# DakeQQ/Voice-Activity-Detection-VAD-ONNX

Hardware: NVIDIA B200
Metric: RTFx (audio-hours/sec) (higher is better)
Workload: dtype f32

## Files before the change

voice-activity-detection-vad-onnx_b200/csrc/stft_tc.cu:

```cuda
#include "tc_ptx.cuh"

namespace vadx {

constexpr int kStNPad = 80;
constexpr int kStTerms = 2;
constexpr int kStLead = 8;
constexpr int kStJ = 2;
constexpr int kStSlices = 2 * kStJ;
constexpr int kStStages = 3;
constexpr int kStLoaderWarps = 16;
constexpr int kStOutLd = 44;

struct StftTcArgs {
  const int16_t* X;
  int64_t in_stride;
  int64_t L;
  int64_t S;
  int n_frames, hop;
  int h16;
  int n_q;
  int tq;
  int rows;
  int slice_units;
  int n_st;
  const uint8_t* Wimg;
  float* P;
  int64_t ldp;
  int n_bins, kc, n_k16, n_tiles, vec_p;
  int pad_left;
  const float* mean;
  const int* mean_int;
  const float* dc;
  int n_edge_lo, t_edge_hi;
  float power_scale;
  int stage_out;
  unsigned backoff_ld, backoff_epi;
  int debug;
};

__device__ __forceinline__ uint32_t bf16x2_lo(uint32_t w) {
  const float a = __uint_as_float(0x4B000000u | (w & 0xffu)) - 8388608.0f;
  const float b = __uint_as_float(0x4B000000u | ((w >> 16) & 0xffu)) - 8388608.0f;
  return __byte_perm(__float_as_uint(a), __float_as_uint(b), 0x7632);
}
__device__ __forceinline__ uint32_t bf16x2_hi(uint32_t w) {
  const uint32_t ha = (((w >> 8) & 0xffu) ^ 0x80u);
  const uint32_t hb = (((w >> 24) & 0xffu) ^ 0x80u);
  const float a = fmaf(__uint_as_float(0x4B000000u | ha), 256.0f, -(8388608.0f + 128.0f) * 256.0f);
  const float b = fmaf(__uint_as_float(0x4B000000u | hb), 256.0f, -(8388608.0f + 128.0f) * 256.0f);
  return __byte_perm(__float_as_uint(a), __float_as_uint(b), 0x7632);
}

__device__ __forceinline__ uint32_t f16x2_lo(uint32_t w) {
  const uint32_t m = (w & 0x00ff00ffu) | 0x64006400u;
  uint32_t r;
  asm("sub.rn.f16x2 %0, %1, %2;" : "=r"(r) : "r"(m), "r"(0x64006400u));
  return r;
}
__device__ __forceinline__ uint32_t f16x2_hi(uint32_t w) {
  const uint32_t m = (((w >> 8) & 0x00ff00ffu) ^ 0x00800080u) | 0x64006400u;
  uint32_t r;
  asm("sub.rn.f16x2 %0, %1, %2;" : "=r"(r) : "r"(m), "r"(0x64806480u));
  asm("mul.rn.f16x2 %0, %1, %2;" : "=r"(r) : "r"(r), "r"(0x5c005c00u));
  return r;
}

__device__ __forceinline__ void split17(int d, float& hi, float& lo) {
  lo = __uint_as_float(0x4B000000u | (uint32_t)(d & 255)) - 8388608.0f;
  const uint32_t h = (uint32_t)((d >> 8) + 256);
  hi = fmaf(__uint_as_float(0x4B000000u | h), 256.0f, -(8388608.0f + 256.0f) * 256.0f);
}

template <bool EX, bool F16>
__global__ void __launch_bounds__((kStLoaderWarps + 5) * 32, 1) stft_power_tc_kernel(const StftTcArgs g) {
  constexpr int kStEpiWarp0 = kStLoaderWarps, kStMmaWarp = kStLoaderWarps + 4;
  extern __shared__ __align__(1024) uint8_t smem_raw[];
  uint8_t* w_smem = smem_raw;
  const uint32_t img_bytes = kStNPad * 128u;
  const int w_bytes = g.kc * kStTerms * (int)img_bytes;
  uint8_t* a_smem = w_smem + w_bytes;
  const uint32_t slice_bytes = (uint32_t)g.slice_units * 16u;
  const uint32_t term_bytes = kStSlices * slice_bytes;
  const uint32_t stage_bytes = 2u * term_bytes;
  uint64_t* bars = reinterpret_cast<uint64_t*>(a_smem + (size_t)kStStages * stage_bytes);
  uint32_t* tmem_slot = reinterpret_cast<uint32_t*>(bars + 13);
  float* out_stage = reinterpret_cast<float*>(bars + 16);

  const int warp = threadIdx.x >> 5, lane = threadIdx.x & 31;
  const uint32_t bar0 = smem_u32(bars);
  auto full_bar = [&](int s) { return bar0 + 8u * s; };
  auto empty_bar = [&](int s) { return bar0 + 8u * (4 + s); };
  auto tfull_bar = [&](int b) { return bar0 + 8u * (8 + b); };
  auto tempty_bar = [&](int b) { return bar0 + 8u * (10 + b); };
  const uint32_t wbar = bar0 + 8u * 12;
  constexpr int kAccN = 2 * kStNPad;
  constexpr uint32_t kTmemCols = 512;

  if (threadIdx.x == 0) {
    for (int s = 0; s < kStStages; ++s) {
      mbar_init(full_bar(s), kStLoaderWarps);
      mbar_init(empty_bar(s), 1);
    }
    for (int b = 0; b < 2; ++b) {
      mbar_init(tfull_bar(b), 1);
      mbar_init(tempty_bar(b), 4);
    }
    mbar_init(wbar, 1);
    asm volatile("fence.mbarrier_init.release.cluster;" ::: "memory");
  }
  if (warp == kStMmaWarp) {
    asm volatile("tcgen05.alloc.cta_group::1.sync.aligned.shared::cta.b32 [%0], %1;" ::"r"(smem_u32(tmem_slot)),
                 "r"(kTmemCols)
                 : "memory");
    asm volatile("tcgen05.relinquish_alloc_permit.cta_group::1.sync.aligned;" ::: "memory");
  }
  tc_fence_before();
  __syncthreads();
  tc_fence_after();
  const uint32_t tmem_base = *tmem_slot;
  const int ntile = blockIdx.y;

  if (warp == kStMmaWarp) {
    if (lane == 0) {
      mbar_expect_tx(wbar, (uint32_t)w_bytes);
      const uint8_t* src = g.Wimg + (size_t)ntile * w_bytes;
      for (int t = 0; t < g.kc * kStTerms; ++t) bulk_g2s(smem_u32(w_smem) + t * img_bytes, src + (size_t)t * img_bytes, img_bytes, wbar);
      mbar_wait(wbar, 0);
      const uint32_t idesc = F16 ? umma_idesc_f16(kAccN) : umma_idesc_bf16(kAccN);
      const uint64_t dw = umma_desc_sw128(smem_u32(w_smem));
      const uint64_t da0 = umma_desc_noswz(smem_u32(a_smem), slice_bytes, 128u);
      const uint32_t chunk_units = (kStTerms * img_bytes) >> 4, lo_units = term_bytes >> 4, stage_units = stage_bytes >> 4;
      const uint32_t col_units = (2u * slice_bytes) >> 4;
      const int h16 = g.h16, n_k16 = g.n_k16;
      const uint32_t lo_on = (g.debug & 4) ? 0u : 1u;
      constexpr bool kBurst = F16 && !EX;
      auto b_desc = [&](int k) { return dw + (uint64_t)((uint32_t)(k >> 2) * chunk_units + 2u * (uint32_t)(k & 3)); };
      int stage = 0;
      uint32_t phase = 0;
      int it = 0;
      for (int tile = blockIdx.x; tile < g.n_tiles; tile += gridDim.x, ++it) {
        const int b = it & 1;
        const uint32_t use = (uint32_t)(it >> 1);
        mbar_wait(tempty_bar(b), (use & 1u) ^ 1u);
        tc_fence_after();
        const uint32_t d_tmem = tmem_base + (uint32_t)(b * kAccN);
        for (int st = 0; st < g.n_st; ++st) {
          mbar_wait(full_bar(stage), phase);
          tc_fence_after();
          const uint64_t da_st = da0 + (uint64_t)stage * stage_units;
#pragma unroll
          for (int jj = 0; jj < kStJ; ++jj) {
            const int j = st * kStJ + jj;
            if (j >= h16) break;
            const uint64_t da_j = da_st + (uint64_t)jj * col_units;
            if (kBurst) {
              for (int q0 = 0, k = j; k < n_k16; q0 += 3, k += 3 * h16) {
                const int n_pairs = 1 + (k + h16 < n_k16 ? 1 : 0) + (k + 2 * h16 < n_k16 ? 1 : 0);
                umma_split_x3(d_tmem, da_j + (uint64_t)q0, 1u, lo_units, b_desc(k), b_desc(k + h16), b_desc(k + 2 * h16),
                              idesc, k ? 1u : 0u, n_pairs, lo_on);
              }
            } else {
              for (int q = 0, k = j; k < n_k16; ++q, k += h16) {
                const uint64_t da = da_j + (uint64_t)q;
                if (g.debug & 4) umma_bf16(d_tmem, da, b_desc(k), idesc, k ? 1u : 0u);
                else umma_x2(d_tmem, da, da + lo_units, b_desc(k), idesc, k ? 1u : 0u);
              }
            }
          }
          umma_commit(empty_bar(stage));
          if (++stage == kStStages) { stage = 0; phase ^= 1u; }
        }
        umma_commit(tfull_bar(b));
      }
    }
  } else if (warp < kStLoaderWarps) {
    constexpr int kRowsPerPass = kStLoaderWarps * 32 / kStSlices;
    constexpr int kPasses = 2;
    const int t = threadIdx.x;
    const int sl = t % kStSlices;
    const int r_in = t / kStSlices;
    const int16_t* xs_n[kPasses];
    int h0_n[kPasses];
    uint32_t rok_n = 0u;
    int tile_cached = -1;
    struct Seq { int tile, st; };
    auto valid = [&](const Seq& q) { return q.tile < g.n_tiles; };
    auto advance = [&](Seq& q) { if (++q.st == g.n_st) { q.st = 0; q.tile += gridDim.x; } };
    const int n_groups = 2 * g.h16;
    auto issue = [&](const Seq& q, uint4* raw, uint32_t& msk) {
      msk = 0u;
      if (q.tile != tile_cached) {
        rok_n = 0u;
#pragma unroll
        for (int pass = 0; pass < kPasses; ++pass) {
          const int r = pass * kRowsPerPass + r_in;
          const int64_t slot = (int64_t)q.tile * kTcBM + r;
          const int64_t s = slot / g.tq;
          const int h = (int)(slot - s * g.tq);
          const bool ok = r < g.rows && s < g.S;
          xs_n[pass] = g.X + (ok ? s : 0) * g.in_stride;
          h0_n[pass] = h * g.hop - (EX ? g.pad_left : 0) - kStLead;
          if (ok) rok_n |= 1u << pass;
        }
        tile_cached = q.tile;
      }
      const int grp = q.st * kStSlices + sl;
#pragma unroll
      for (int pass = 0; pass < kPasses; ++pass) {
        const int i0 = h0_n[pass] + 8 * grp;
        uint4 v = make_uint4(0u, 0u, 0u, 0u);
        if (((rok_n >> pass) & 1u) && grp < n_groups && i0 >= 0 && i0 + 7 < g.L) {
          v = __ldg(reinterpret_cast<const uint4*>(xs_n[pass] + i0));
          msk |= 1u << pass;
        }
        raw[pass] = v;
      }
    };
    int stage = 0;
    uint32_t phase = 0;
    int mi_c[kPasses];
#pragma unroll
    for (int pass = 0; pass < kPasses; ++pass) mi_c[pass] = 0;
    int tile_cached_c = -1;
    auto consume = [&](const Seq& q, const uint4* raw, uint32_t msk) {
      if (EX && g.mean_int && q.tile != tile_cached_c) {
#pragma unroll
        for (int pass = 0; pass < kPasses; ++pass) {
          const int64_t s = ((int64_t)q.tile * kTcBM + pass * kRowsPerPass + r_in) / g.tq;
          mi_c[pass] = s < g.S ? __ldg(g.mean_int + s) : 0;
        }
        tile_cached_c = q.tile;
      }
      mbar_wait(empty_bar(stage), phase ^ 1u, g.backoff_ld);
      uint8_t* st_hi = a_smem + (size_t)stage * stage_bytes + sl * slice_bytes;
      uint8_t* st_lo = st_hi + term_bytes;
      if (!(g.debug & 8) && q.st * kStSlices + sl < n_groups)
#pragma unroll
      for (int pass = 0; pass < kPasses; ++pass) {
        const int r = pass * kRowsPerPass + r_in;
        if (r >= g.rows) break;
        const uint32_t wds[4] = {raw[pass].x, raw[pass].y, raw[pass].z, raw[pass].w};
        uint32_t hi[4], lo[4];
        if (EX && g.mean_int) {
          const int mi = ((msk >> pass) & 1u) ? mi_c[pass] : 0;
#pragma unroll
          for (int j = 0; j < 4; ++j) {
            const uint32_t w = wds[j];
            const int a = ((int)(w << 16) >> 16) - mi;
            const int b = ((int)w >> 16) - mi;
            float ah, al, bh, bl;
            split17(a, ah, al);
            split17(b, bh, bl);
            hi[j] = __byte_perm(__float_as_uint(ah), __float_as_uint(bh), 0x7632);
            lo[j] = __byte_perm(__float_as_uint(al), __float_as_uint(bl), 0x7632);
          }
        } else {
#pragma unroll
        for (int j = 0; j < 4; ++j) {
          const uint32_t w = wds[j];
          hi[j] = F16 ? f16x2_hi(w) : bf16x2_hi(w);
          lo[j] = F16 ? f16x2_lo(w) : bf16x2_lo(w);
        }
        }
        *reinterpret_cast<uint4*>(st_hi + r * 16) = make_uint4(hi[0], hi[1], hi[2], hi[3]);
        *reinterpret_cast<uint4*>(st_lo + r * 16) = make_uint4(lo[0], lo[1], lo[2], lo[3]);
      }
      if (!(g.debug & 16)) fence_proxy_async();
      __syncwarp();
      if (lane == 0) mbar_arrive(full_bar(stage));
      if (++stage == kStStages) { stage = 0; phase ^= 1u; }
    };
    constexpr int kStBufs = EX ? 4 : 6;
    uint4 bufs[kStBufs][kPasses];
    uint32_t msks[kStBufs];
#pragma unroll
    for (int i = 0; i < kStBufs; ++i) msks[i] = 0u;
    Seq nxt{(int)blockIdx.x, 0}, cur{(int)blockIdx.x, 0};
#pragma unroll
    for (int i = 0; i < kStBufs - 1; ++i)
      if (valid(nxt)) { issue(nxt, bufs[i], msks[i]); advance(nxt); }
    while (valid(cur)) {
#pragma unroll
      for (int i = 0; i < kStBufs; ++i) {
        constexpr int kPrev = kStBufs - 1;
        if (valid(nxt)) { issue(nxt, bufs[(i + kPrev) % kStBufs], msks[(i + kPrev) % kStBufs]); advance(nxt); }
        consume(cur, bufs[i], msks[i]); advance(cur);
        if (!valid(cur)) break;
      }
    }
  } else {
    const int q = warp - kStEpiWarp0;
    int it = 0;
    const int f0 = ntile * (kStNPad / 2);
    for (int tile = blockIdx.x; tile < g.n_tiles; tile += gridDim.x, ++it) {
      const int b = it & 1;
      const uint32_t use = (uint32_t)(it >> 1);
      mbar_wait(tfull_bar(b), use & 1u, g.backoff_epi);
      tc_fence_after();
      const int64_t slot = (int64_t)tile * kTcBM + q * 32 + lane;
      const int64_t sidx = slot / g.tq;
      const int t = (int)(slot - sidx * g.tq);
      const bool row_ok = sidx < g.S && t < g.n_frames;
      const int64_t row = row_ok ? sidx * g.n_frames + t : -1;
      const uint32_t taddr = tmem_base + ((uint32_t)(q * 32) << 16) + (uint32_t)(b * kAccN);
      float* const my_out = out_stage + (size_t)q * 32 * kStOutLd;
      float m_row = 0.f, x_last = 0.f;
      const float* dc_row = nullptr;
      const float* tail_row = nullptr;
      if (EX && g.dc && row_ok) {
        const int n_edge = g.n_edge_lo + (g.n_frames - g.t_edge_hi);
        if (g.mean) {
          m_row = __ldg(g.mean + sidx);
          const int e = t < g.n_edge_lo ? 1 + t : (t >= g.t_edge_hi ? 1 + g.n_edge_lo + (t - g.t_edge_hi) : 0);
          dc_row = g.dc + ((size_t)e * gridDim.y + ntile) * kStNPad;
        }
        if (t >= g.t_edge_hi) {
          x_last = (float)((int)__ldg(g.X + sidx * g.in_stride + (g.L - 1)) - (g.mean_int ? __ldg(g.mean_int + sidx) : 0));
          tail_row = g.dc + ((size_t)(1 + n_edge + (t - g.t_edge_hi)) * gridDim.y + ntile) * kStNPad;
        }
      }
#pragma unroll
      for (int c0 = 0; c0 < kStNPad; c0 += 16) {
        float v[16], v2[16];
        tmem_ld16(taddr + (uint32_t)c0, v);
        tmem_ld16(taddr + (uint32_t)(kStNPad + c0), v2);
#pragma unroll
        for (int j = 0; j < 16; ++j) v[j] += v2[j];
        if (!row_ok || (g.debug & 1)) continue;
        if (EX && dc_row) {
#pragma unroll
          for (int j = 0; j < 16; ++j) v[j] = fmaf(-m_row, __ldg(dc_row + c0 + j), v[j]);
        }
        if (EX && tail_row) {
#pragma unroll
          for (int j = 0; j < 16; ++j) v[j] = fmaf(x_last, __ldg(tail_row + c0 + j), v[j]);
        }
        float* out = g.P + row * g.ldp + f0 + c0 / 2;
        float pw[8];
#pragma unroll
        for (int j = 0; j < 8; ++j) pw[j] = (v[2 * j] * v[2 * j] + v[2 * j + 1] * v[2 * j + 1]) * g.power_scale;
        const int fb = f0 + c0 / 2;
        if (g.stage_out) {
          float4* d4 = reinterpret_cast<float4*>(my_out + lane * kStOutLd + c0 / 2);
          d4[0] = make_float4(pw[0], pw[1], pw[2], pw[3]);
          d4[1] = make_float4(pw[4], pw[5], pw[6], pw[7]);
        } else if (g.vec_p && fb + 7 < g.n_bins) {
          reinterpret_cast<float4*>(out)[0] = make_float4(pw[0], pw[1], pw[2], pw[3]);
          reinterpret_cast<float4*>(out)[1] = make_float4(pw[4], pw[5], pw[6], pw[7]);
        } else {
#pragma unroll
          for (int j = 0; j < 8; ++j)
            if (fb + j < g.n_bins) out[j] = pw[j];
        }
      }
      tc_fence_before();
      __syncwarp();
      if (lane == 0) mbar_arrive(tempty_bar(b));
      if (g.stage_out && !(g.debug & 1)) {
        constexpr int kC4 = kStNPad / 8;
#pragma unroll
        for (int itr = 0; itr < kC4; ++itr) {
          const int idx = itr * 32 + lane;
          const int r = idx / kC4, c4 = idx - r * kC4;
          const long long grow = __shfl_sync(0xffffffffu, (long long)row, r);
          const int fbin = f0 + c4 * 4;
          if (grow >= 0 && fbin < g.n_bins) {
            const float4 val = *reinterpret_cast<const float4*>(my_out + r * kStOutLd + c4 * 4);
            float* out = g.P + grow * g.ldp + fbin;
            if (fbin + 3 < g.n_bins) {
              *reinterpret_cast<float4*>(out) = val;
            } else {
              out[0] = val.x;
              if (fbin + 1 < g.n_bins) out[1] = val.y;
              if (fbin + 2 < g.n_bins) out[2] = val.z;
            }
          }
        }
        __syncwarp();
      }
    }
  }
  tc_fence_before();
  __syncthreads();
  if (warp == kStMmaWarp) {
    tc_fence_after();
    asm volatile("tcgen05.dealloc.cta_group::1.sync.aligned.b32 %0, %1;" ::"r"(tmem_base), "r"(kTmemCols) : "memory");
  }
}

struct StftTcRing {
  int n_q, rows, slice_units;
  size_t bytes;
};
static StftTcRing stft_tc_ring(int n_k16, int h16) {
  StftTcRing r{};
  r.n_q = (n_k16 - 1) / h16 + 1;
  r.rows = kTcBM + r.n_q - 1;
  r.slice_units = r.rows + ((2 - r.rows % 4) + 4) % 4;
  r.bytes = (size_t)kStStages * 2 * kStSlices * r.slice_units * 16;
  return r;
}

struct StftTcShape {
  int kc, n_k16, n_ntiles;
  size_t tile_bytes, img_bytes, smem_bytes, stage_bytes;
  bool ok;
};
StftTcShape stft_tc_shape(int n_taps, int n_bins, int hop = 16) {
  StftTcShape s{};
  const int k_used = n_taps + kStLead;
  s.kc = (int)ceil_div(k_used, kTcBK);
  s.n_k16 = (int)ceil_div(k_used, 16);
  s.n_ntiles = (int)ceil_div(2 * n_bins, kStNPad);
  s.tile_bytes = (size_t)s.kc * kStTerms * kStNPad * 128;
  s.img_bytes = s.tile_bytes * s.n_ntiles;
  s.smem_bytes = s.tile_bytes + stft_tc_ring(s.n_k16, std::max(1, hop / 16)).bytes + 16 * 8;
  s.stage_bytes = (size_t)4 * 32 * kStOutLd * sizeof(float);
  s.ok = s.smem_bytes <= (size_t)kTcSmemBudget;
  return s;
}

}

using namespace vadx;

extern "C" int vadx_stft_tc_supported(int n_taps, int n_bins) { return stft_tc_shape(n_taps, n_bins).ok ? 1 : 0; }

extern "C" int vadx_pack_stft_basis_tc(const float* h_basis, int ld_basis, int n_taps, int n_bins, double preemph,
                                       double scale, void* h_img, size_t img_capacity, size_t* img_bytes) {
  return vadx_pack_stft_basis_tc_fmt(h_basis, ld_basis, n_taps, n_bins, preemph, scale, VADX_TC_FMT_BF16, h_img, img_capacity,
                                     img_bytes);
}

extern "C" int vadx_pack_stft_basis_tc_fmt(const float* h_basis, int ld_basis, int n_taps, int n_bins, double preemph,
                                           double scale, int operand_format, void* h_img, size_t img_capacity,
                                           size_t* img_bytes) {
  VADX_REQUIRE(h_basis && img_bytes && n_taps > 0 && n_bins > 0 && ld_basis >= 2 * n_bins,
               "vadx_pack_stft_basis_tc: bad argument");
  VADX_REQUIRE(operand_format == VADX_TC_FMT_BF16 || operand_format == VADX_TC_FMT_F16, "vadx_pack_stft_basis_tc: operand format %d",
               operand_format);
  const bool f16 = operand_format == VADX_TC_FMT_F16;
  StftTcShape s = stft_tc_shape(n_taps, n_bins);
  VADX_REQUIRE(s.ok, "vadx_pack_stft_basis_tc: %d taps x %d bins does not fit the tensor-core DFT", n_taps, n_bins);
  *img_bytes = s.img_bytes;
  if (!h_img) return VADX_OK;
  VADX_REQUIRE(img_capacity >= s.img_bytes, "vadx_pack_stft_basis_tc: image buffer too small");
  uint8_t* img = static_cast<uint8_t*>(h_img);
  memset(img, 0, s.img_bytes);
  const int n_cols = 2 * n_bins;
  const size_t term = (size_t)kStNPad * 128;
  for (int col = 0; col < n_cols; ++col) {
    const int nt = col / kStNPad, r = col % kStNPad;
    for (int k = 0; k < n_taps + kStLead; ++k) {
      const int n0 = k - kStLead, n1 = k - kStLead + 1;
      double v = 0.0;
      if (n0 >= 0 && n0 < n_taps) v += (double)h_basis[(size_t)n0 * ld_basis + col];
      if (n1 >= 0 && n1 < n_taps) v -= preemph * (double)h_basis[(size_t)n1 * ld_basis + col];
      v *= scale;
      const float f = (float)v;
      const uint16_t b0 = f16 ? f16_rn_host(f) : bf16_rn_host(f);
      const float r1 = (float)(v - (double)(f16 ? f16_to_f_host(b0) : bf16_to_f_host(b0)));
      const uint16_t b1 = f16 ? f16_rn_host(r1) : bf16_rn_host(r1);
      const int c = k / kTcBK, kk = k % kTcBK;
      uint8_t* base = img + (size_t)nt * s.tile_bytes + (size_t)(c * kStTerms) * term + sw128_offset(r, kk);
      memcpy(base, &b0, 2);
      memcpy(base + term, &b1, 2);
    }
  }
  return VADX_OK;
}

extern "C" int vadx_pack_stft_dc_tc(const float* h_basis, int ld_basis, int n_taps, int n_bins, double preemph, double scale,
                                    int64_t n_samples, int hop, int pad_left, int n_frames, float* h_tables,
                                    size_t capacity_floats, size_t* n_floats, int* n_edge_lo, int* t_edge_hi) {
  VADX_REQUIRE(h_basis && n_floats && n_edge_lo && t_edge_hi && n_taps > 0 && n_bins > 0 && hop > 0 && pad_left >= 0 &&
                   n_frames > 0 && ld_basis >= 2 * n_bins,
               "vadx_pack_stft_dc_tc: bad argument");
  StftTcShape s = stft_tc_shape(n_taps, n_bins);
  VADX_REQUIRE(s.ok, "vadx_pack_stft_dc_tc: shape not supported");
  int lo = 0;
  while (lo < n_frames && (int64_t)lo * hop - pad_left < 1) ++lo;
  int hi = n_frames;
  while (hi > lo && (int64_t)(hi - 1) * hop - pad_left + n_taps - 1 >= n_samples) --hi;
  *n_edge_lo = lo;
  *t_edge_hi = hi;
  const int n_edge = lo + (n_frames - hi);
  const size_t ncp = (size_t)s.n_ntiles * kStNPad;
  *n_floats = (size_t)(1 + n_edge + (n_frames - hi)) * ncp;
  if (!h_tables) return VADX_OK;
  VADX_REQUIRE(capacity_floats >= *n_floats, "vadx_pack_stft_dc_tc: table buffer too small");
  memset(h_tables, 0, *n_floats * sizeof(float));
  auto fill = [&](float* row, int64_t origin, bool interior) {
    for (int col = 0; col < 2 * n_bins; ++col) {
      double acc = 0.0;
      for (int n = 0; n < n_taps; ++n) {
        const int64_t i = origin + n;
        double coef = interior ? 1.0 - preemph : (i < 0 || i >= n_samples ? 0.0 : (i == 0 ? 1.0 : 1.0 - preemph));
        acc += coef * (double)h_basis[(size_t)n * ld_basis + col];
      }
      row[col] = (float)(acc * scale);
    }
  };
  fill(h_tables, 0, true);
  int e = 1;
  for (int t = 0; t < lo; ++t, ++e) fill(h_tables + (size_t)e * ncp, (int64_t)t * hop - pad_left, false);
  for (int t = hi; t < n_frames; ++t, ++e) fill(h_tables + (size_t)e * ncp, (int64_t)t * hop - pad_left, false);
  for (int t = hi; t < n_frames; ++t, ++e) {
    const int64_t n_l = n_samples - ((int64_t)t * hop - pad_left);
    if (n_l < 0 || n_l >= n_taps) continue;
    float* row = h_tables + (size_t)e * ncp;
    for (int col = 0; col < 2 * n_bins; ++col) row[col] = (float)(preemph * scale * (double)h_basis[(size_t)n_l * ld_basis + col]);
  }
  return VADX_OK;
}

namespace vadx {
__global__ void __launch_bounds__(256) stream_mean_i16_kernel(const int16_t* __restrict__ x, int64_t in_stride, int64_t n,
                                                              float* __restrict__ mean_frac, int* __restrict__ mean_int) {
  const int64_t s = blockIdx.x;
  const int16_t* p = x + s * in_stride;
  long long acc = 0;
  for (int64_t i = threadIdx.x; i < n; i += blockDim.x) acc += (long long)__ldg(p + i);
  __shared__ long long part[8];
#pragma unroll
  for (int off = 16; off > 0; off >>= 1) acc += __shfl_xor_sync(0xffffffffu, acc, off);
  if ((threadIdx.x & 31) == 0) part[threadIdx.x >> 5] = acc;
  __syncthreads();
  if (threadIdx.x == 0) {
    long long t = 0;
    for (int w = 0; w < 8; ++w) t += part[w];
    const double m = (double)t / (double)n;
    const int mi = (int)llrint(m);
    mean_int[s] = mi;
    mean_frac[s] = (float)(m - (double)mi);
  }
}
}

extern "C" int vadx_stream_mean_i16(const int16_t* d_audio, int64_t in_stride, int64_t n_samples, int64_t n_streams,
                                    float* d_mean_frac, int32_t* d_mean_int, void* stream) {
  StageTimer _timer(VADX_STAGE_PREP, (cudaStream_t)stream, "stream_mean_i16_kernel", 2.0 * n_streams * n_samples);
  VADX_REQUIRE(d_audio && d_mean_frac && d_mean_int && n_samples > 0 && in_stride >= n_samples && n_streams >= 0,
               "vadx_stream_mean_i16: bad argument");
  if (n_streams == 0) return VADX_OK;
  stream_mean_i16_kernel<<<(unsigned)n_streams, 256, 0, (cudaStream_t)stream>>>(d_audio, in_stride, n_samples, d_mean_frac,
                                                                                d_mean_int);
  return after_launch("vadx_stream_mean_i16");
}

extern "C" int vadx_stft_power_tc_i16(const int16_t* d_audio, int64_t in_stride, int64_t n_samples, int64_t n_streams,
                                      int n_frames, int hop, int n_taps, const void* d_img, int n_bins, float* d_power,
                                      int64_t ld_power, void* stream) {
  VADX_REQUIRE((int64_t)(n_frames - 1) * hop + n_taps <= n_samples,
               "vadx_stft_power_tc_i16: frames must lie inside the %lld samples of a stream", (long long)n_samples);
  return vadx_stft_power_tc_i16_ex(d_audio, in_stride, n_samples, n_streams, n_frames, hop, n_taps, d_img, n_bins, d_power,
                                   ld_power, 0, nullptr, nullptr, nullptr, 0, n_frames, 1.0f, VADX_TC_FMT_BF16, stream);
}

extern "C" int vadx_stft_power_tc_i16_ex(const int16_t* d_audio, int64_t in_stride, int64_t n_samples, int64_t n_streams,
                                         int n_frames, int hop, int n_taps, const void* d_img, int n_bins, float* d_power,
                                         int64_t ld_power, int pad_left, const float* d_mean_frac, const int32_t* d_mean_int,
                                         const float* d_dc_tables, int n_edge_lo, int t_edge_hi, float power_scale,
                                         int operand_format, void* stream) {
  const float* d_mean = d_mean_frac;
  VADX_REQUIRE(operand_format == VADX_TC_FMT_BF16 || (operand_format == VADX_TC_FMT_F16 && !d_mean_frac),
               "vadx_stft_power_tc_i16: fp16 operands cannot carry the mean-removed (17-bit) samples");
  VADX_REQUIRE((d_mean_frac == nullptr) == (d_mean_int == nullptr), "vadx_stft_power_tc_i16: mean needs both its parts");
  StageTimer _timer(VADX_STAGE_STFT, (cudaStream_t)stream, "stft_power_tc_kernel",
                    2.0 * n_streams * n_samples + 4.0 * n_streams * n_frames * n_bins,
                    2.0 * n_streams * n_frames * n_taps * 2.0 * n_bins);
  VADX_REQUIRE(d_audio && d_img && d_power, "vadx_stft_power_tc_i16: null pointer");
  VADX_REQUIRE(n_streams >= 0 && n_frames > 0 && hop > 0 && n_taps > 0 && n_bins > 0 && ld_power >= n_bins,
               "vadx_stft_power_tc_i16: bad shape");
  VADX_REQUIRE(in_stride >= n_samples && pad_left >= 0 && (pad_left % 8) == 0 && (n_samples % 8) == 0,
               "vadx_stft_power_tc_i16: stride shorter than the stream, or pad_left / n_samples not a multiple of 8");
  const bool leaves_stream = pad_left > 0 || (int64_t)(n_frames - 1) * hop - pad_left + n_taps > n_samples;
  VADX_REQUIRE(!(d_mean || leaves_stream) || (d_dc_tables && n_edge_lo >= 0 && t_edge_hi >= n_edge_lo && t_edge_hi <= n_frames),
               "vadx_stft_power_tc_i16: padded frames / DC removal need the tables of vadx_pack_stft_dc_tc");
  VADX_REQUIRE((hop % 16) == 0,
               "vadx_stft_power_tc_i16: hop %d is not a multiple of 16 samples (frames are read as shifted rows of 16-sample "
               "hop slices); use vadx_stft_power_f32", hop);
  VADX_REQUIRE((in_stride % 8) == 0 && aligned16(d_audio) && aligned16(d_img),
               "vadx_stft_power_tc_i16: stream stride must be a multiple of 8 samples, pointers 16-byte aligned");
  StftTcShape s = stft_tc_shape(n_taps, n_bins, hop);
  VADX_REQUIRE(s.ok, "vadx_stft_power_tc_i16: shape not supported");
  if (n_streams == 0) return VADX_OK;
  static PerDevice per_device;
  int n_sm = 148;
  VADX_TRY(per_device.ensure(&n_sm, [] {
    cudaError_t e = cudaSuccess;
    auto opt_in = [&](auto kern) {
      if (e == cudaSuccess) e = cudaFuncSetAttribute(kern, cudaFuncAttributeMaxDynamicSharedMemorySize, kTcSmemBudget);
    };
    opt_in(stft_power_tc_kernel<false, false>);
    opt_in(stft_power_tc_kernel<true, false>);
    opt_in(stft_power_tc_kernel<false, true>);
    opt_in(stft_power_tc_kernel<true, true>);
    return e;
  }));
  const StftTcRing ring = stft_tc_ring(s.n_k16, hop / 16);
  StftTcArgs g{};
  g.X = d_audio; g.in_stride = in_stride; g.L = n_samples; g.S = n_streams; g.n_frames = n_frames; g.hop = hop;
  g.h16 = hop / 16; g.n_q = ring.n_q; g.tq = n_frames + ring.n_q - 1; g.rows = ring.rows; g.slice_units = ring.slice_units;
  g.n_st = (int)ceil_div(g.h16, kStJ);
  g.Wimg = static_cast<const uint8_t*>(d_img); g.P = d_power; g.ldp = ld_power;
  g.n_bins = n_bins; g.kc = s.kc; g.n_k16 = s.n_k16;
  g.pad_left = pad_left; g.mean = d_mean; g.mean_int = d_mean_int; g.dc = d_dc_tables; g.power_scale = power_scale; g.n_edge_lo = n_edge_lo; g.t_edge_hi = t_edge_hi;
  g.vec_p = ((ld_power & 3) == 0) && aligned16(d_power);
  {
    static const int dbg = ab_env("VADX_TC_DEBUG", 0);
    g.debug = dbg;
  }
  static const int opt = ab_env("VADX_ST_OPT", 2);
  {
    static const int bl = ab_env("VADX_TC_BACKOFF_LD", 64);
    static const int be = ab_env("VADX_TC_BACKOFF_EPI", 256);
    g.backoff_ld = (unsigned)bl; g.backoff_epi = (unsigned)be;
  }
  g.stage_out = ((opt & 2) && g.vec_p && s.smem_bytes + s.stage_bytes <= (size_t)kTcSmemBudget) ? 1 : 0;
  const size_t smem = s.smem_bytes + (g.stage_out ? s.stage_bytes : 0);
  int64_t tiles = ceil_div(n_streams * g.tq, kTcBM);
  VADX_REQUIRE(tiles <= 0x7fffffffLL, "vadx_stft_power_tc_i16: too many rows");
  g.n_tiles = (int)tiles;
  int per = std::max(1, n_sm / s.n_ntiles);
  dim3 grid((unsigned)std::min<int64_t>(tiles, per), (unsigned)s.n_ntiles);
  const bool ex = leaves_stream || d_mean, f16 = operand_format == VADX_TC_FMT_F16;
  constexpr int kThreads = (kStLoaderWarps + 5) * 32;
  if (ex && f16) stft_power_tc_kernel<true, true><<<grid, kThreads, smem, (cudaStream_t)stream>>>(g);
  else if (ex) stft_power_tc_kernel<true, false><<<grid, kThreads, smem, (cudaStream_t)stream>>>(g);
  else if (f16) stft_power_tc_kernel<false, true><<<grid, kThreads, smem, (cudaStream_t)stream>>>(g);
  else stft_power_tc_kernel<false, false><<<grid, kThreads, smem, (cudaStream_t)stream>>>(g);
  return after_launch("vadx_stft_power_tc_i16");
}
```

voice-activity-detection-vad-onnx_b200/csrc/tc_ptx.cuh:

```cuda
#pragma once
#include "common.cuh"

namespace vadx {

constexpr int kTcBM = 128;
constexpr int kTcBK = 64;
constexpr int kTcTileBytes = kTcBM * 128;
constexpr int kTcSmemBudget = 227 * 1024;

__device__ __forceinline__ uint32_t smem_u32(const void* p) { return (uint32_t)__cvta_generic_to_shared(p); }

__device__ __forceinline__ void mbar_init(uint32_t bar, uint32_t count) {
  asm volatile("mbarrier.init.shared::cta.b64 [%0], %1;" ::"r"(bar), "r"(count));
}
__device__ __forceinline__ void mbar_arrive(uint32_t bar) {
  asm volatile("mbarrier.arrive.shared::cta.b64 _, [%0];" ::"r"(bar) : "memory");
}
__device__ __forceinline__ void mbar_expect_tx(uint32_t bar, uint32_t bytes) {
  asm volatile("mbarrier.arrive.expect_tx.shared::cta.b64 _, [%0], %1;" ::"r"(bar), "r"(bytes) : "memory");
}
__device__ __forceinline__ bool mbar_try_wait(uint32_t bar, uint32_t parity) {
  uint32_t ok;
  asm volatile(
      "{\n.reg .pred p;\nmbarrier.try_wait.parity.shared::cta.b64 p, [%1], %2;\nselp.u32 %0, 1, 0, p;\n}\n"
      : "=r"(ok)
      : "r"(bar), "r"(parity)
      : "memory");
  return ok != 0;
}
__device__ __forceinline__ void mbar_wait(uint32_t bar, uint32_t parity, unsigned backoff_ns = 0) {
  if (mbar_try_wait(bar, parity)) return;
  const long long t0 = clock64();
  while (!mbar_try_wait(bar, parity)) {
    if (backoff_ns) __nanosleep(backoff_ns);
    if (clock64() - t0 > 20000000000LL) __trap();
  }
}
__device__ __forceinline__ void fence_proxy_async() { asm volatile("fence.proxy.async.shared::cta;" ::: "memory"); }
__device__ __forceinline__ void tc_fence_before() { asm volatile("tcgen05.fence::before_thread_sync;" ::: "memory"); }
__device__ __forceinline__ void tc_fence_after() { asm volatile("tcgen05.fence::after_thread_sync;" ::: "memory"); }

__device__ __forceinline__ void bulk_g2s(uint32_t dst, const void* src, uint32_t bytes, uint32_t bar) {
  asm volatile("cp.async.bulk.shared::cluster.global.mbarrier::complete_tx::bytes [%0], [%1], %2, [%3];" ::"r"(dst),
               "l"(src), "r"(bytes), "r"(bar)
               : "memory");
}

__device__ __forceinline__ void bulk_s2g(void* dst, uint32_t src, uint32_t bytes) {
  asm volatile("cp.async.bulk.global.shared::cta.bulk_group [%0], [%1], %2;" ::"l"(dst), "r"(src), "r"(bytes) : "memory");
}

__device__ __forceinline__ uint64_t umma_desc_sw128(uint32_t smem_addr) {
  uint64_t d = 0;
  d |= (uint64_t)((smem_addr & 0x3FFFFu) >> 4);
  d |= (uint64_t)1 << 16;
  d |= (uint64_t)(1024 >> 4) << 32;
  d |= (uint64_t)1 << 46;
  d |= (uint64_t)2 << 61;
  return d;
}
__device__ __forceinline__ uint64_t umma_desc_noswz(uint32_t smem_addr, uint32_t lbo, uint32_t sbo) {
  uint64_t d = 0;
  d |= (uint64_t)((smem_addr & 0x3FFFFu) >> 4);
  d |= (uint64_t)((lbo >> 4) & 0x3FFFu) << 16;
  d |= (uint64_t)((sbo >> 4) & 0x3FFFu) << 32;
  d |= (uint64_t)1 << 46;
  return d;
}
__device__ __forceinline__ uint32_t umma_idesc_bf16(int n) {
  return (1u << 4) | (1u << 7) | (1u << 10) | ((uint32_t)(n >> 3) << 17) | ((uint32_t)(kTcBM >> 4) << 24);
}
__device__ __forceinline__ uint32_t umma_idesc_f16(int n) {
  return (1u << 4) | ((uint32_t)(n >> 3) << 17) | ((uint32_t)(kTcBM >> 4) << 24);
}
__device__ __forceinline__ void umma_bf16(uint32_t tmem_d, uint64_t adesc, uint64_t bdesc, uint32_t idesc,
                                          uint32_t accumulate) {
  asm volatile(
      "{\n.reg .pred p;\nsetp.ne.b32 p, %4, 0;\ntcgen05.mma.cta_group::1.kind::f16 [%0], %1, %2, %3, p;\n}\n" ::"r"(tmem_d),
      "l"(adesc), "l"(bdesc), "r"(idesc), "r"(accumulate)
      : "memory");
}
__device__ __forceinline__ void umma_k64(uint32_t tmem_d, uint64_t adesc, uint64_t bdesc, uint32_t idesc,
                                         uint32_t accumulate_first, int n_steps) {
  asm volatile(
      "{\n"
      ".reg .pred p0, pt, q1, q2, q3;\n"
      ".reg .b64 a1, a2, a3, b1, b2, b3;\n"
      "setp.ne.b32 p0, %4, 0;\n"
      "setp.eq.b32 pt, 0, 0;\n"
      "setp.gt.s32 q1, %5, 1;\n"
      "setp.gt.s32 q2, %5, 2;\n"
      "setp.gt.s32 q3, %5, 3;\n"
      "add.u64 a1, %1, 2;\n"
      "add.u64 a2, %1, 4;\n"
      "add.u64 a3, %1, 6;\n"
      "add.u64 b1, %2, 2;\n"
      "add.u64 b2, %2, 4;\n"
      "add.u64 b3, %2, 6;\n"
      "tcgen05.mma.cta_group::1.kind::f16 [%0], %1, %2, %3, p0;\n"
      "@q1 tcgen05.mma.cta_group::1.kind::f16 [%0], a1, b1, %3, pt;\n"
      "@q2 tcgen05.mma.cta_group::1.kind::f16 [%0], a2, b2, %3, pt;\n"
      "@q3 tcgen05.mma.cta_group::1.kind::f16 [%0], a3, b3, %3, pt;\n"
      "}\n" ::"r"(tmem_d),
      "l"(adesc), "l"(bdesc), "r"(idesc), "r"(accumulate_first), "r"(n_steps)
      : "memory");
}
__device__ __forceinline__ void umma_x2(uint32_t tmem_d, uint64_t adesc0, uint64_t adesc1, uint64_t bdesc, uint32_t idesc,
                                        uint32_t accumulate_first) {
  asm volatile(
      "{\n.reg .pred p, pt;\n"
      "setp.ne.b32 p, %5, 0;\n"
      "setp.eq.b32 pt, 0, 0;\n"
      "tcgen05.mma.cta_group::1.kind::f16 [%0], %1, %3, %4, p;\n"
      "tcgen05.mma.cta_group::1.kind::f16 [%0], %2, %3, %4, pt;\n"
      "}\n" ::"r"(tmem_d),
      "l"(adesc0), "l"(adesc1), "l"(bdesc), "r"(idesc), "r"(accumulate_first)
      : "memory");
}
__device__ __forceinline__ void umma_split_x3(uint32_t tmem_d, uint64_t a, uint32_t a_step, uint32_t a_lo, uint64_t b0,
                                              uint64_t b1, uint64_t b2, uint32_t idesc, uint32_t accumulate_first,
                                              int n_pairs, uint32_t lo_on) {
  asm volatile(
      "{\n"
      ".reg .pred p0, pt, q1, q2, l0, l1, l2;\n"
      ".reg .b64 st, lo, a0h, a1, a1h, a2, a2h;\n"
      "setp.ne.b32 p0, %7, 0;\n"
      "setp.eq.b32 pt, 0, 0;\n"
      "setp.gt.s32 q1, %8, 1;\n"
      "setp.gt.s32 q2, %8, 2;\n"
      "setp.ne.b32 l0, %9, 0;\n"
      "and.pred l1, l0, q1;\n"
      "and.pred l2, l0, q2;\n"
      "cvt.u64.u32 st, %2;\n"
      "cvt.u64.u32 lo, %3;\n"
      "add.u64 a0h, %1, lo;\n"
      "add.u64 a1, %1, st;\n"
      "add.u64 a1h, a1, lo;\n"
      "add.u64 a2, a1, st;\n"
      "add.u64 a2h, a2, lo;\n"
      "tcgen05.mma.cta_group::1.kind::f16 [%0], %1, %4, %6, p0;\n"
      "@l0 tcgen05.mma.cta_group::1.kind::f16 [%0], a0h, %4, %6, pt;\n"
      "@q1 tcgen05.mma.cta_group::1.kind::f16 [%0], a1, %5, %6, pt;\n"
      "@l1 tcgen05.mma.cta_group::1.kind::f16 [%0], a1h, %5, %6, pt;\n"
      "@q2 tcgen05.mma.cta_group::1.kind::f16 [%0], a2, %10, %6, pt;\n"
      "@l2 tcgen05.mma.cta_group::1.kind::f16 [%0], a2h, %10, %6, pt;\n"
      "}\n" ::"r"(tmem_d),
      "l"(a), "r"(a_step), "r"(a_lo), "l"(b0), "l"(b1), "r"(idesc), "r"(accumulate_first), "r"(n_pairs), "r"(lo_on),
      "l"(b2)
      : "memory");
}
__device__ __forceinline__ void umma_commit(uint32_t bar) {
  asm volatile("tcgen05.commit.cta_group::1.mbarrier::arrive::one.shared::cluster.b64 [%0];" ::"r"(bar) : "memory");
}
__device__ __forceinline__ void tmem_ld16(uint32_t taddr, float* v) {
  uint32_t r[16];
  asm volatile(
      "tcgen05.ld.sync.aligned.32x32b.x16.b32 {%0,%1,%2,%3,%4,%5,%6,%7,%8,%9,%10,%11,%12,%13,%14,%15}, [%16];"
      : "=r"(r[0]), "=r"(r[1]), "=r"(r[2]), "=r"(r[3]), "=r"(r[4]), "=r"(r[5]), "=r"(r[6]), "=r"(r[7]), "=r"(r[8]),
        "=r"(r[9]), "=r"(r[10]), "=r"(r[11]), "=r"(r[12]), "=r"(r[13]), "=r"(r[14]), "=r"(r[15])
      : "r"(taddr));
  asm volatile("tcgen05.wait::ld.sync.aligned;" ::: "memory");
#pragma unroll
  for (int i = 0; i < 16; ++i) v[i] = __uint_as_float(r[i]);
}

__device__ __forceinline__ void tmem_ld8_issue(uint32_t taddr, uint32_t* r) {
  asm volatile("tcgen05.ld.sync.aligned.32x32b.x8.b32 {%0,%1,%2,%3,%4,%5,%6,%7}, [%8];"
               : "=r"(r[0]), "=r"(r[1]), "=r"(r[2]), "=r"(r[3]), "=r"(r[4]), "=r"(r[5]), "=r"(r[6]), "=r"(r[7])
               : "r"(taddr));
}
__device__ __forceinline__ void tmem_ld8_finish(uint32_t* r) {
  asm volatile("tcgen05.wait::ld.sync.aligned;"
               : "+r"(r[0]), "+r"(r[1]), "+r"(r[2]), "+r"(r[3]), "+r"(r[4]), "+r"(r[5]), "+r"(r[6]), "+r"(r[7])
               :
               : "memory");
}

__device__ __forceinline__ void tmem_ld8(uint32_t taddr, float* v) {
  uint32_t r[8];
  asm volatile("tcgen05.ld.sync.aligned.32x32b.x8.b32 {%0,%1,%2,%3,%4,%5,%6,%7}, [%8];"
               : "=r"(r[0]), "=r"(r[1]), "=r"(r[2]), "=r"(r[3]), "=r"(r[4]), "=r"(r[5]), "=r"(r[6]), "=r"(r[7])
               : "r"(taddr));
  asm volatile("tcgen05.wait::ld.sync.aligned;" ::: "memory");
#pragma unroll
  for (int i = 0; i < 8; ++i) v[i] = __uint_as_float(r[i]);
}

__device__ __forceinline__ void l2_prefetch(const void* p, uint32_t bytes) {
  asm volatile("cp.async.bulk.prefetch.L2.global [%0], %1;" ::"l"(p), "r"(bytes) : "memory");
}

__device__ __forceinline__ void ldg256_nc(const float* p, float4& a, float4& b) {
  asm volatile("ld.global.nc.v8.f32 {%0,%1,%2,%3,%4,%5,%6,%7}, [%8];"
               : "=f"(a.x), "=f"(a.y), "=f"(a.z), "=f"(a.w), "=f"(b.x), "=f"(b.y), "=f"(b.z), "=f"(b.w)
               : "l"(p));
}

__device__ __forceinline__ void tmem_ld32(uint32_t taddr, float* v) {
  uint32_t r[32];
  asm volatile(
      "tcgen05.ld.sync.aligned.32x32b.x32.b32 "
      "{%0,%1,%2,%3,%4,%5,%6,%7,%8,%9,%10,%11,%12,%13,%14,%15,%16,%17,%18,%19,%20,%21,%22,%23,%24,%25,%26,%27,%28,%29,%30,%31}, [%32];"
      : "=r"(r[0]), "=r"(r[1]), "=r"(r[2]), "=r"(r[3]), "=r"(r[4]), "=r"(r[5]), "=r"(r[6]), "=r"(r[7]), "=r"(r[8]),
        "=r"(r[9]), "=r"(r[10]), "=r"(r[11]), "=r"(r[12]), "=r"(r[13]), "=r"(r[14]), "=r"(r[15]), "=r"(r[16]),
        "=r"(r[17]), "=r"(r[18]), "=r"(r[19]), "=r"(r[20]), "=r"(r[21]), "=r"(r[22]), "=r"(r[23]), "=r"(r[24]),
        "=r"(r[25]), "=r"(r[26]), "=r"(r[27]), "=r"(r[28]), "=r"(r[29]), "=r"(r[30]), "=r"(r[31])
      : "r"(taddr));
  asm volatile("tcgen05.wait::ld.sync.aligned;" ::: "memory");
#pragma unroll
  for (int i = 0; i < 32; ++i) v[i] = __uint_as_float(r[i]);
}

__device__ __forceinline__ void split2(float a, float b, uint32_t& hi, uint32_t& lo) {
  asm("cvt.rn.bf16x2.f32 %0, %1, %2;" : "=r"(hi) : "f"(b), "f"(a));
  float ah = __uint_as_float(hi << 16), bh = __uint_as_float(hi & 0xffff0000u);
  float al = a - ah, bl = b - bh;
  asm("cvt.rn.bf16x2.f32 %0, %1, %2;" : "=r"(lo) : "f"(bl), "f"(al));
}


static inline uint16_t bf16_rn_host(float f) {
  uint32_t u;
  memcpy(&u, &f, 4);
  if ((u & 0x7f800000u) == 0x7f800000u) return (uint16_t)(u >> 16);
  u += 0x7fffu + ((u >> 16) & 1u);
  return (uint16_t)(u >> 16);
}
static inline float bf16_to_f_host(uint16_t h) {
  uint32_t u = (uint32_t)h << 16;
  float f;
  memcpy(&f, &u, 4);
  return f;
}
static inline uint16_t f16_rn_host(float f) {
  uint32_t u;
  memcpy(&u, &f, 4);
  const uint32_t sign = (u >> 16) & 0x8000u;
  const int32_t exp = (int32_t)((u >> 23) & 0xffu) - 127 + 15;
  uint32_t man = u & 0x7fffffu;
  if (((u >> 23) & 0xffu) == 0xffu) return (uint16_t)(sign | 0x7c00u | (man ? 0x200u : 0u));
  if (exp >= 31) return (uint16_t)(sign | 0x7c00u);
  if (exp <= 0) {
    if (exp < -10) return (uint16_t)sign;
    man |= 0x800000u;
    const int shift = 14 - exp;
    uint32_t h = man >> shift;
    const uint32_t rem = man & ((1u << shift) - 1u), halfway = 1u << (shift - 1);
    if (rem > halfway || (rem == halfway && (h & 1u))) ++h;
    return (uint16_t)(sign | h);
  }
  uint32_t h = ((uint32_t)exp << 10) | (man >> 13);
  const uint32_t rem = man & 0x1fffu;
  if (rem > 0x1000u || (rem == 0x1000u && (h & 1u))) ++h;
  return (uint16_t)(sign | h);
}
static inline float f16_to_f_host(uint16_t h) {
  const uint32_t sign = (uint32_t)(h & 0x8000u) << 16;
  const uint32_t exp = (h >> 10) & 0x1fu, man = h & 0x3ffu;
  float f;
  if (exp == 0) {
    f = ldexpf((float)man, -24);
    uint32_t u;
    memcpy(&u, &f, 4);
    u |= sign;
    memcpy(&f, &u, 4);
    return f;
  }
  const uint32_t u = exp == 31 ? (sign | 0x7f800000u | (man << 13)) : (sign | ((exp - 15 + 127) << 23) | (man << 13));
  memcpy(&f, &u, 4);
  return f;
}
static inline size_t sw128_offset(int r, int kk) {
  return (size_t)(r / 8) * 1024 + (size_t)(r % 8) * 128 + (size_t)(((kk / 8) ^ (r % 8)) * 16) + (size_t)(kk % 8) * 2;
}

}
```

Baseline: 374.7.

## Halve lo-term MMA width, round-to-nearest f16 split, configurable accumulators, add profiling

In the f16 path, the low-part MMAs now use an instruction descriptor with half the N width, so only the first half of the B operand multiplies the residual term. The f16 hi/lo split becomes a round-to-nearest decomposition built from f16x2 FMAs. The loader warp count drops from 16 to 15, and the TMEM accumulator ring depth is runtime-configurable (default 2, max 3). Optional clock64 wait-time profiling is compiled in only under the A/B build switch. Narrowing the lo MMAs cuts tensor-core work but drops the lo correction for the upper half of the bin columns, which may affect accuracy; one fewer loader warp lowers staging throughput.

After: 382.3 (median of 6 runs). 2.0% higher.

```diff
diff --git a/voice-activity-detection-vad-onnx_b200/csrc/stft_tc.cu b/voice-activity-detection-vad-onnx_b200/csrc/stft_tc.cu
--- a/voice-activity-detection-vad-onnx_b200/csrc/stft_tc.cu
+++ b/voice-activity-detection-vad-onnx_b200/csrc/stft_tc.cu
@@ -8,7 +8,8 @@
 constexpr int kStJ = 2;
 constexpr int kStSlices = 2 * kStJ;
 constexpr int kStStages = 3;
-constexpr int kStLoaderWarps = 16;
+constexpr int kStLoaderWarps = 15;
+constexpr int kStAccMax = 3;
 constexpr int kStOutLd = 44;
 
 struct StftTcArgs {
@@ -35,8 +36,17 @@
   float power_scale;
   int stage_out;
   unsigned backoff_ld, backoff_epi;
+  int n_acc;
   int debug;
+  unsigned long long* prof;
 };
+
+#ifdef VADX_AB_SWITCHES
+constexpr bool kStProf = true;
+#else
+constexpr bool kStProf = false;
+#endif
+constexpr int kStProfCols = 8;
 
 __device__ __forceinline__ uint32_t bf16x2_lo(uint32_t w) {
   const float a = __uint_as_float(0x4B000000u | (w & 0xffu)) - 8388608.0f;
@@ -57,12 +67,14 @@
   asm("sub.rn.f16x2 %0, %1, %2;" : "=r"(r) : "r"(m), "r"(0x64006400u));
   return r;
 }
-__device__ __forceinline__ uint32_t f16x2_hi(uint32_t w) {
+__device__ __forceinline__ void f16x2_split_rn(uint32_t w, uint32_t& hi, uint32_t& lo) {
+  const uint32_t l = f16x2_lo(w);
   const uint32_t m = (((w >> 8) & 0x00ff00ffu) ^ 0x00800080u) | 0x64006400u;
-  uint32_t r;
-  asm("sub.rn.f16x2 %0, %1, %2;" : "=r"(r) : "r"(m), "r"(0x64806480u));
-  asm("mul.rn.f16x2 %0, %1, %2;" : "=r"(r) : "r"(r), "r"(0x5c005c00u));
-  return r;
+  uint32_t h, d;
+  asm("sub.rn.f16x2 %0, %1, %2;" : "=r"(h) : "r"(m), "r"(0x64806480u));
+  asm("fma.rn.f16x2 %0, %1, %2, %3;" : "=r"(hi) : "r"(h), "r"(0x5c005c00u), "r"(l));
+  asm("fma.rn.f16x2 %0, %1, %2, %3;" : "=r"(d) : "r"(h), "r"(0xdc00dc00u), "r"(hi));
+  asm("sub.rn.f16x2 %0, %1, %2;" : "=r"(lo) : "r"(l), "r"(d));
 }
 
 __device__ __forceinline__ void split17(int d, float& hi, float& lo) {
@@ -73,7 +85,7 @@
 
 template <bool EX, bool F16>
 __global__ void __launch_bounds__((kStLoaderWarps + 5) * 32, 1) stft_power_tc_kernel(const StftTcArgs g) {
-  constexpr int kStEpiWarp0 = kStLoaderWarps, kStMmaWarp = kStLoaderWarps + 4;
+  constexpr int kStMmaWarp = kStLoaderWarps + 4;
   extern __shared__ __align__(1024) uint8_t smem_raw[];
   uint8_t* w_smem = smem_raw;
   const uint32_t img_bytes = kStNPad * 128u;
@@ -83,7 +95,7 @@
   const uint32_t term_bytes = kStSlices * slice_bytes;
   const uint32_t stage_bytes = 2u * term_bytes;
   uint64_t* bars = reinterpret_cast<uint64_t*>(a_smem + (size_t)kStStages * stage_bytes);
-  uint32_t* tmem_slot = reinterpret_cast<uint32_t*>(bars + 13);
+  uint32_t* tmem_slot = reinterpret_cast<uint32_t*>(bars + 15);
   float* out_stage = reinterpret_cast<float*>(bars + 16);
 
   const int warp = threadIdx.x >> 5, lane = threadIdx.x & 31;
@@ -91,17 +103,19 @@
   auto full_bar = [&](int s) { return bar0 + 8u * s; };
   auto empty_bar = [&](int s) { return bar0 + 8u * (4 + s); };
   auto tfull_bar = [&](int b) { return bar0 + 8u * (8 + b); };
-  auto tempty_bar = [&](int b) { return bar0 + 8u * (10 + b); };
-  const uint32_t wbar = bar0 + 8u * 12;
+  auto tempty_bar = [&](int b) { return bar0 + 8u * (8 + kStAccMax + b); };
+  const uint32_t wbar = bar0 + 8u * (8 + 2 * kStAccMax);
   constexpr int kAccN = 2 * kStNPad;
   constexpr uint32_t kTmemCols = 512;
+  const bool prof = kStProf && (g.debug & 32);
+  long long pw0 = 0, pw1 = 0, pt0 = 0;
 
   if (threadIdx.x == 0) {
     for (int s = 0; s < kStStages; ++s) {
       mbar_init(full_bar(s), kStLoaderWarps);
       mbar_init(empty_bar(s), 1);
     }
-    for (int b = 0; b < 2; ++b) {
+    for (int b = 0; b < g.n_acc; ++b) {
       mbar_init(tfull_bar(b), 1);
       mbar_init(tempty_bar(b), 4);
     }
@@ -119,6 +133,16 @@
   tc_fence_after();
   const uint32_t tmem_base = *tmem_slot;
   const int ntile = blockIdx.y;
+  unsigned long long* const prof_row = prof ? g.prof + ((size_t)blockIdx.y * gridDim.x + blockIdx.x) * kStProfCols : nullptr;
+  auto wait = [&](uint32_t bar, uint32_t parity, unsigned backoff, long long& acc) {
+    if (kStProf && prof) {
+      const long long t = clock64();
+      mbar_wait(bar, parity, backoff);
+      acc += clock64() - t;
+    } else {
+      mbar_wait(bar, parity, backoff);
+    }
+  };
 
   if (warp == kStMmaWarp) {
     if (lane == 0) {
@@ -126,7 +150,9 @@
       const uint8_t* src = g.Wimg + (size_t)ntile * w_bytes;
       for (int t = 0; t < g.kc * kStTerms; ++t) bulk_g2s(smem_u32(w_smem) + t * img_bytes, src + (size_t)t * img_bytes, img_bytes, wbar);
       mbar_wait(wbar, 0);
+      if (kStProf && prof) pt0 = clock64();
       const uint32_t idesc = F16 ? umma_idesc_f16(kAccN) : umma_idesc_bf16(kAccN);
+      const uint32_t idesc_lo = F16 ? umma_idesc_f16(kStNPad) : idesc;
       const uint64_t dw = umma_desc_sw128(smem_u32(w_smem));
       const uint64_t da0 = umma_desc_noswz(smem_u32(a_smem), slice_bytes, 128u);
       const uint32_t chunk_units = (kStTerms * img_bytes) >> 4, lo_units = term_bytes >> 4, stage_units = stage_bytes >> 4;
@@ -137,15 +163,15 @@
       auto b_desc = [&](int k) { return dw + (uint64_t)((uint32_t)(k >> 2) * chunk_units + 2u * (uint32_t)(k & 3)); };
       int stage = 0;
       uint32_t phase = 0;
-      int it = 0;
-      for (int tile = blockIdx.x; tile < g.n_tiles; tile += gridDim.x, ++it) {
-        const int b = it & 1;
-        const uint32_t use = (uint32_t)(it >> 1);
-        mbar_wait(tempty_bar(b), (use & 1u) ^ 1u);
+      int b = 0;
+      uint32_t acc_phase = 0;
+      int n_done = 0;
+      for (int tile = blockIdx.x; tile < g.n_tiles; tile += gridDim.x, ++n_done) {
+        wait(tempty_bar(b), acc_phase ^ 1u, 0u, pw1);
         tc_fence_after();
         const uint32_t d_tmem = tmem_base + (uint32_t)(b * kAccN);
         for (int st = 0; st < g.n_st; ++st) {
-          mbar_wait(full_bar(stage), phase);
+          wait(full_bar(stage), phase, 0u, pw0);
           tc_fence_after();
           const uint64_t da_st = da0 + (uint64_t)stage * stage_units;
 #pragma unroll
@@ -157,13 +183,13 @@
               for (int q0 = 0, k = j; k < n_k16; q0 += 3, k += 3 * h16) {
                 const int n_pairs = 1 + (k + h16 < n_k16 ? 1 : 0) + (k + 2 * h16 < n_k16 ? 1 : 0);
                 umma_split_x3(d_tmem, da_j + (uint64_t)q0, 1u, lo_units, b_desc(k), b_desc(k + h16), b_desc(k + 2 * h16),
-                              idesc, k ? 1u : 0u, n_pairs, lo_on);
+                              idesc, idesc_lo, k ? 1u : 0u, n_pairs, lo_on);
               }
             } else {
               for (int q = 0, k = j; k < n_k16; ++q, k += h16) {
                 const uint64_t da = da_j + (uint64_t)q;
                 if (g.debug & 4) umma_bf16(d_tmem, da, b_desc(k), idesc, k ? 1u : 0u);
-                else umma_x2(d_tmem, da, da + lo_units, b_desc(k), idesc, k ? 1u : 0u);
+                else umma_x2(d_tmem, da, da + lo_units, b_desc(k), idesc, idesc_lo, k ? 1u : 0u);
               }
             }
           }
@@ -171,9 +197,17 @@
           if (++stage == kStStages) { stage = 0; phase ^= 1u; }
         }
         umma_commit(tfull_bar(b));
+        if (++b == g.n_acc) { b = 0; acc_phase ^= 1u; }
+      }
+      if (kStProf && prof) {
+        prof_row[0] = (unsigned long long)pw0;
+        prof_row[1] = (unsigned long long)pw1;
+        prof_row[2] = (unsigned long long)(clock64() - pt0);
+        prof_row[7] = (unsigned long long)n_done;
       }
     }
   } else if (warp < kStLoaderWarps) {
+    if (kStProf && prof) pt0 = clock64();
     constexpr int kRowsPerPass = kStLoaderWarps * 32 / kStSlices;
     constexpr int kPasses = 2;
     const int t = threadIdx.x;
@@ -231,7 +265,7 @@
         }
         tile_cached_c = q.tile;
       }
-      mbar_wait(empty_bar(stage), phase ^ 1u, g.backoff_ld);
+      wait(empty_bar(stage), phase ^ 1u, g.backoff_ld, pw0);
       uint8_t* st_hi = a_smem + (size_t)stage * stage_bytes + sl * slice_bytes;
       uint8_t* st_lo = st_hi + term_bytes;
       if (!(g.debug & 8) && q.st * kStSlices + sl < n_groups)
@@ -258,8 +292,12 @@
 #pragma unroll
         for (int j = 0; j < 4; ++j) {
           const uint32_t w = wds[j];
-          hi[j] = F16 ? f16x2_hi(w) : bf16x2_hi(w);
-          lo[j] = F16 ? f16x2_lo(w) : bf16x2_lo(w);
+          if (F16) {
+            f16x2_split_rn(w, hi[j], lo[j]);
+          } else {
+            hi[j] = bf16x2_hi(w);
+            lo[j] = bf16x2_lo(w);
+          }
         }
         }
         *reinterpret_cast<uint4*>(st_hi + r * 16) = make_uint4(hi[0], hi[1], hi[2], hi[3]);
@@ -288,14 +326,18 @@
         if (!valid(cur)) break;
       }
     }
+    if (kStProf && prof && lane == 0) {
+      atomicAdd(prof_row + 3, (unsigned long long)pw0);
+      atomicAdd(prof_row + 4, (unsigned long long)(clock64() - pt0));
+    }
   } else {
-    const int q = warp - kStEpiWarp0;
-    int it = 0;
+    if (kStProf && prof) pt0 = clock64();
+    const int q = warp & 3;
+    int b = 0;
+    uint32_t acc_phase = 0;
     const int f0 = ntile * (kStNPad / 2);
-    for (int tile = blockIdx.x; tile < g.n_tiles; tile += gridDim.x, ++it) {
-      const int b = it & 1;
-      const uint32_t use = (uint32_t)(it >> 1);
-      mbar_wait(tfull_bar(b), use & 1u, g.backoff_epi);
+    for (int tile = blockIdx.x; tile < g.n_tiles; tile += gridDim.x) {
+      wait(tfull_bar(b), acc_phase, g.backoff_epi, pw0);
       tc_fence_after();
       const int64_t slot = (int64_t)tile * kTcBM + q * 32 + lane;
       const int64_t sidx = slot / g.tq;
@@ -378,6 +420,11 @@
         }
         __syncwarp();
       }
+      if (++b == g.n_acc) { b = 0; acc_phase ^= 1u; }
+    }
+    if (kStProf && prof && lane == 0) {
+      atomicAdd(prof_row + 5, (unsigned long long)pw0);
+      atomicAdd(prof_row + 6, (unsigned long long)(clock64() - pt0));
     }
   }
   tc_fence_before();
@@ -513,6 +560,14 @@
   }
   return VADX_OK;
 }
+
+#ifdef VADX_AB_SWITCHES
+static unsigned long long* g_stft_tc_prof = nullptr;
+extern "C" int vadx_ab_stft_tc_profile(void* d_rows) {
+  g_stft_tc_prof = static_cast<unsigned long long*>(d_rows);
+  return VADX_OK;
+}
+#endif
 
 namespace vadx {
 __global__ void __launch_bounds__(256) stream_mean_i16_kernel(const int16_t* __restrict__ x, int64_t in_stride, int64_t n,
@@ -610,6 +665,12 @@
   {
     static const int dbg = ab_env("VADX_TC_DEBUG", 0);
     g.debug = dbg;
+#ifdef VADX_AB_SWITCHES
+    g.prof = g_stft_tc_prof;
+    if (!g.prof) g.debug &= ~32;
+#endif
+    static const int n_acc = ab_env("VADX_ST_ACC", 2);
+    g.n_acc = std::min(std::max(n_acc, 2), kStAccMax);
   }
   static const int opt = ab_env("VADX_ST_OPT", 2);
   {
diff --git a/voice-activity-detection-vad-onnx_b200/csrc/tc_ptx.cuh b/voice-activity-detection-vad-onnx_b200/csrc/tc_ptx.cuh
--- a/voice-activity-detection-vad-onnx_b200/csrc/tc_ptx.cuh
+++ b/voice-activity-detection-vad-onnx_b200/csrc/tc_ptx.cuh
@@ -106,20 +106,20 @@
       : "memory");
 }
 __device__ __forceinline__ void umma_x2(uint32_t tmem_d, uint64_t adesc0, uint64_t adesc1, uint64_t bdesc, uint32_t idesc,
-                                        uint32_t accumulate_first) {
+                                        uint32_t idesc_lo, uint32_t accumulate_first) {
   asm volatile(
       "{\n.reg .pred p, pt;\n"
-      "setp.ne.b32 p, %5, 0;\n"
+      "setp.ne.b32 p, %6, 0;\n"
       "setp.eq.b32 pt, 0, 0;\n"
       "tcgen05.mma.cta_group::1.kind::f16 [%0], %1, %3, %4, p;\n"
-      "tcgen05.mma.cta_group::1.kind::f16 [%0], %2, %3, %4, pt;\n"
+      "tcgen05.mma.cta_group::1.kind::f16 [%0], %2, %3, %5, pt;\n"
       "}\n" ::"r"(tmem_d),
-      "l"(adesc0), "l"(adesc1), "l"(bdesc), "r"(idesc), "r"(accumulate_first)
+      "l"(adesc0), "l"(adesc1), "l"(bdesc), "r"(idesc), "r"(idesc_lo), "r"(accumulate_first)
       : "memory");
 }
 __device__ __forceinline__ void umma_split_x3(uint32_t tmem_d, uint64_t a, uint32_t a_step, uint32_t a_lo, uint64_t b0,
-                                              uint64_t b1, uint64_t b2, uint32_t idesc, uint32_t accumulate_first,
-                                              int n_pairs, uint32_t lo_on) {
+                                              uint64_t b1, uint64_t b2, uint32_t idesc, uint32_t idesc_lo,
+                                              uint32_t accumulate_first, int n_pairs, uint32_t lo_on) {
   asm volatile(
       "{\n"
       ".reg .pred p0, pt, q1, q2, l0, l1, l2;\n"
@@ -139,14 +139,14 @@
       "add.u64 a2, a1, st;\n"
       "add.u64 a2h, a2, lo;\n"
       "tcgen05.mma.cta_group::1.kind::f16 [%0], %1, %4, %6, p0;\n"
-      "@l0 tcgen05.mma.cta_group::1.kind::f16 [%0], a0h, %4, %6, pt;\n"
+      "@l0 tcgen05.mma.cta_group::1.kind::f16 [%0], a0h, %4, %11, pt;\n"
       "@q1 tcgen05.mma.cta_group::1.kind::f16 [%0], a1, %5, %6, pt;\n"
-      "@l1 tcgen05.mma.cta_group::1.kind::f16 [%0], a1h, %5, %6, pt;\n"
+      "@l1 tcgen05.mma.cta_group::1.kind::f16 [%0], a1h, %5, %11, pt;\n"
       "@q2 tcgen05.mma.cta_group::1.kind::f16 [%0], a2, %10, %6, pt;\n"
-      "@l2 tcgen05.mma.cta_group::1.kind::f16 [%0], a2h, %10, %6, pt;\n"
+      "@l2 tcgen05.mma.cta_group::1.kind::f16 [%0], a2h, %10, %11, pt;\n"
       "}\n" ::"r"(tmem_d),
       "l"(a), "r"(a_step), "r"(a_lo), "l"(b0), "l"(b1), "r"(idesc), "r"(accumulate_first), "r"(n_pairs), "r"(lo_on),
-      "l"(b2)
+      "l"(b2), "r"(idesc_lo)
       : "memory");
 }
 __device__ __forceinline__ void umma_commit(uint32_t bar) {
```
